# DiltheyLab/HLA-LA

Hardware: AMD Instinct MI355X
Metric: paired reads/sec aligned to PRG graph (higher is better)
Workload: dtype int32

## Files before the change

### hla-la_amd/__init__.py

```python
from __future__ import annotations

import ctypes as C
import os

import numpy as np

_HERE = os.path.dirname(os.path.abspath(__file__))
LIB_PATH = os.environ.get("HLALA_LIB_PATH") or os.path.join(_HERE, "libhlala_gpu.so")

c_i32p = C.POINTER(C.c_int32)
c_i64p = C.POINTER(C.c_int64)
c_u8p = C.POINTER(C.c_uint8)
c_u32p = C.POINTER(C.c_uint32)
c_f64p = C.POINTER(C.c_double)

CHAIN_OK, CHAIN_SKIP_STRAND, CHAIN_SKIP_DUP = 0, 1, 2
CHAIN_ERR_COLUMNS, CHAIN_ERR_FRONTIER, CHAIN_ERR_INPUT = -1, -2, -3


class GraphDesc(C.Structure):
    _fields_ = [("n_levels", C.c_int32), ("n_nodes", C.c_int32), ("n_edges", C.c_int32),
                ("node_level", c_i32p), ("edge_from", c_i32p), ("edge_to", c_i32p), ("edge_label", c_u8p)]


# ... 946 lines not shown
EXPORTED_SYMBOLS = [
    "hlala_debug_work_counters", "hlala_debug_dp_items", "hlala_debug_counters", "hlala_debug_buffer", "hlala_debug_memory",
    "hlala_set_tail_pool", "hlala_flush",
    "hlala_set_pair_overflow", "hlala_get_pair_overflow", "hlala_pair_overflow_need", "hlala_batch_get_pair_overflow",
    "hlala_comm_create", "hlala_comm_destroy", "hlala_comm_uses_rccl", "hlala_comm_last_error", "hlala_gather_pair_records", "hlala_reduce_coverage",
    "hlala_create", "hlala_destroy", "hlala_last_error", "hlala_graph_get_info", "hlala_graph_get_nodes",
    "hlala_graph_get_paths", "hlala_graph_get_gap_stretch", "hlala_batch_create",
    "hlala_batch_create_from_seeds", "hlala_batch_create_unpaired", "hlala_batch_set_first_chain", "hlala_batch_destroy", "hlala_project_chains", "hlala_extend_chains",
    "hlala_pair_chains", "hlala_align_batch", "hlala_batch_get_chains", "hlala_batch_get_pairs",
    "hlala_batch_get_stats", "hlala_batch_get_pairs_packed", "hlala_batch_export_pair_records", "hlala_set_gene_intervals", "hlala_postprocess_pairs", "hlala_get_coverage", "hlala_exon_loglik", "hlala_pair_loglik", "hlala_kat_phred",
    "hlala_kat_rand_r", "hlala_kat_exp", "hlala_abi_sizeof", "hlala_abi_version", "hlala_build_flags", "hlala_pack_bases", "hlala_call_locus", "hlala_exon_positions", "hlala_filter_positions", "hlala_estimate_insert_size", "hlala_graph_load_text", "hlala_graph_cache_save",
    "hlala_graph_cache_load", "hlala_graph_file_desc", "hlala_graph_file_free", "hlala_loader_last_error",
    "hlala_bam_extract_seeds", "hlala_bam_extract_seeds_mt", "hlala_bam_extract_seeds_opt", "hlala_seed_batch_counts", "hlala_seed_batch_desc", "hlala_seed_batch_window", "hlala_seed_batch_units", "hlala_seed_batch_name", "hlala_seed_batch_timing",
    "hlala_seed_batch_free", "hlala_seed_batch_pin", "hlala_bam_last_error", "hlala_bam_inflate_engine", "hlala_pinned_alloc", "hlala_pinned_free", "hlala_host_register", "hlala_host_unregister", "hlala_set_insert_size",
    "hlala_contigs_load_dir", "hlala_contigs_open_dir", "hlala_contigs_load_translations", "hlala_contigs_file_desc", "hlala_contigs_file_intervals", "hlala_contigs_file_free",
    "hlala_typer_open", "hlala_typer_close", "hlala_typer_last_error", "hlala_typer_n_levels", "hlala_typer_level_name", "hlala_typer_level_of", "hlala_typer_n_genes",
    "hlala_typer_gene", "hlala_typer_load_g_groups", "hlala_typer_g_translate", "hlala_typer_locus", "hlala_locus_free", "hlala_locus_get", "hlala_locus_cluster_id", "hlala_locus_type_cluster",
    "hlala_inflater_create", "hlala_inflater_destroy", "hlala_inflater_last_error", "hlala_bgzf_inflate", "hlala_bam_extract_seeds_gpu", "hlala_seed_batch_inflate_counts",
    "hlala_bgzf_inflate_crc", "hlala_seed_batch_crc_counts",
    "hlala_bam_scan", "hlala_bam_scan_status_text", "hlala_seed_batch_parse_counts", "hlala_seed_batch_transfer_bytes",
    "hlala_bam_group", "hlala_bam_group_rounds", "hlala_seed_batch_group_counts",
    "hlala_bam_name_order", "hlala_seed_batch_sort_counts",
    "hlala_bam_fill_create", "hlala_bam_fill_window", "hlala_bam_fill_last_error", "hlala_bam_fill_destroy", "hlala_seed_batch_fill_counts", "hlala_seed_batch_fill_ms",
    "hlala_batch_create_from_fill", "hlala_debug_batch_inputs",
    "hlala_locus_cluster_kmers", "hlala_type_locus", "hlala_kmer_presence", "hlala_kmer_keep_reads", "hlala_kmer_presence_kept", "hlala_kmer_forget_reads", "hlala_unit_alignment_stats", "hlala_typer_write_summary", "hlala_typer_begin_output", "hlala_locus_write_files", "hlala_locus_write_pairs_file", "hlala_typer_end_output",
]


PAIR_OVERFLOW_WAVES = 64


def pair_overflow_need(n1, n2, max_columns, unpaired=False):
    lib = load_library()
    lib.hlala_pair_overflow_need.argtypes = [C.c_int64, C.c_int64, C.c_int32, C.c_int]
    lib.hlala_pair_overflow_need.restype = C.c_int64
    return int(lib.hlala_pair_overflow_need(int(n1), int(n2), int(max_columns), int(bool(unpaired))))


class Context:

    def __init__(self, graph: dict, contigs: dict | None, insert_mean=200.0, insert_sd=35.0, rng_seed=12345,
                 long_read_mode=0, max_columns=384, device=0, stream=None):
        self.lib = load_library()
        self.max_columns = max_columns
        g, self._kg = fill_struct(GraphDesc, graph)
        self.params = Params(insert_mean, insert_sd, rng_seed, long_read_mode, max_columns, 0)
        h = C.c_void_p()
# ... 389 lines not shown
```

### hla-la_amd/csrc/hlala_api.hip

```cpp
#include <cmath>
#include <cstdio>
#include <cstring>
#include <cstdlib>
#include <algorithm>
#include <atomic>
#include <map>
#include <mutex>
#include <chrono>
#include <thread>
#include <set>
#include <string>
#include <unordered_map>
#include <vector>

#include "../../include/hlala_gpu.h"
#include "batch.h"
#include "flat_graph.hpp"
#include "host_internal.h"

#include "kernel_dp.hip"
#include "kernel_project.hip"
#include "kernel_order.hip"
#include "kernel_pair.hip"
#include "kernel_pair_overflow.hip"
// ... 14 lines not shown
size_t proj_slab_bytes_host(int stride, int maxNodesPerLevel) { return proj_slab_bytes(stride, maxNodesPerLevel); }
}

using namespace hlala;

static thread_local std::string g_create_error;

struct DevBuf {
    void* p = nullptr; size_t bytes = 0;
};

struct DpClass {
    int grid = 0, block = 0;
    char* slabs = nullptr; size_t slab_bytes = 0;
    const char* name = "";
    void (*launch)(hlala_ctx* c, const DpClass& k, hipStream_t ws, hlala_batch* b, const DpPoolArgs& pool) = nullptr;
};

struct hlala_ctx {
    int device = 0;
    hipStream_t stream = nullptr;
    hipStream_t side = nullptr;
    hipStream_t up = nullptr, rs = nullptr, active = nullptr;
    int tail_pool_k = 1; std::vector<hlala_batch*> tail;
    hipEvent_t evSideTail = nullptr; bool sideTailValid = false;
    hlala_params params{};
    FlatGraph F;
    DevGraph G{};
    DevGraph* dG = nullptr;
    DevTables* dT = nullptr;
    double* d_islog = nullptr;
    long long* d_contig_off = nullptr; uint8_t* d_contig_seq = nullptr; int* d_contig_level = nullptr;
    int n_contigs = 0; std::vector<long long> contig_off;
    std::vector<void*> allocs;
    std::unordered_map<void*, size_t> block_bytes;
    std::multimap<size_t, void*> pool;
    size_t pool_bytes = 0;
    size_t pool_cap = (size_t)176 << 30;
    std::mutex pool_mu;
    std::set<struct hlala_batch*> batches;
    int dp_long_bases = 48;
    int jf_margin = 16;
    int stitch_by_row = 1;
    int stitch_draw = 12;
    bool side_after_pair = false;
    bool rows_all = false;
// ... 145 lines not shown
    auto it = c->pool.lower_bound(bytes);
    if(it != c->pool.end() && it->first <= bytes + bytes / 4 + 4096) {
        *out = it->second; c->pool_bytes -= it->first; c->pool.erase(it);
        return 0;
    }
    void* p = nullptr;
    hipError_t e = device_malloc_retry(c->device, c, &p, bytes);
    if(e != hipSuccess) { c->err = std::string("hipMalloc: ") + hipGetErrorString(e); return HLALA_E_DEVICE; }
    c->block_bytes[p] = bytes;
    *out = p;
    return 0;
}
static void pool_release(hlala_ctx* c, void* p)
{
    if(!p) return;
    std::lock_guard<std::mutex> g(c->pool_mu);
    auto it = c->block_bytes.find(p);
    if(it == c->block_bytes.end()) { (void)hipFree(p); return; }
    if(c->pool_bytes + it->second > c->pool_cap) { c->block_bytes.erase(it); (void)hipFree(p); return; }
    c->pool.emplace(it->second, p); c->pool_bytes += it->second;
}

constexpr size_t PIN_GRANULE = (size_t)64 << 20;
template <class T>
static int dev_upload(hlala_ctx* c, std::vector<void*>& allocs, const T* host, size_t n, T** out)
{
    *out = nullptr;
    size_t bytes = (n ? n : 1) * sizeof(T);
    void* p = nullptr;
    { int rc_ = pool_malloc(c, &p, bytes); if(rc_) return rc_; }
    allocs.push_back(p);
    if(n && host) {
        const char* src = (const char*)host; char* dst = (char*)p; size_t left = n * sizeof(T);
        while(left) {
            const size_t toEdge = PIN_GRANULE - (size_t)((uintptr_t)src & (PIN_GRANULE - 1)), k = left < toEdge ? left : toEdge;
            HIP_TRY(c, hipMemcpyAsync(dst, src, k, hipMemcpyHostToDevice, c->active));
            src += k; dst += k; left -= k;
        }
    }
    *out = (T*)p;
    return 0;
}
template <class T>
static int dev_alloc(hlala_ctx* c, std::vector<void*>& allocs, size_t n, T** out, bool zero = false)
{
    *out = nullptr;
// ... 209 lines not shown
    c->proj_slab_bytes = proj_slab_bytes_host(c->params.max_columns, F.max_nodes_per_level);
    if(device_malloc_retry(c->device, nullptr, (void**)&c->proj_slabs, c->proj_slab_bytes * (size_t)c->proj_grid) != hipSuccess) { c->err = "hipMalloc(projection slabs) failed"; return fail(HLALA_E_DEVICE); }
    c->allocs.push_back(c->proj_slabs);
    if(!c->proj_long_slabs) {
        const char* e = getenv("HLALA_RETHREAD");
        if(!(e && atoi(e) == 0)) {
            size_t ent = (size_t)c->params.max_columns * (size_t)RT_SN; if(ent < 1024) ent = 1024;
            c->rethread_slab_bytes = (ent * sizeof(ChoiceRec) + 255) & ~(size_t)255;
            if(c->rethread_slab_bytes > c->proj_slab_bytes) c->rethread_slab_bytes = c->proj_slab_bytes;
            c->rethread_grid = cus * 24;
            if(device_malloc_retry(c->device, nullptr, (void**)&c->rethread_slabs, c->rethread_slab_bytes * (size_t)c->rethread_grid) != hipSuccess) { c->err = "hipMalloc(re-threading slabs) failed"; return fail(HLALA_E_DEVICE); }
            c->allocs.push_back(c->rethread_slabs);
        }
    }
    { const char* e = getenv("HLALA_LOCALITY");
      if(!(e && atoi(e) == 0)) { int sh = 8; if(e && atoi(e) >= 2 && atoi(e) <= 20) sh = atoi(e); while((F.L >> sh) + 2 > 16384) sh++; c->order_shift = sh; c->order_nb = (F.L >> sh) + 2; } }
    if(const char* e = getenv("HLALA_LONG_CHUNK_NODES")) { const int v = atoi(e); if(v >= 1) c->long_chunk_nodes = v; }
    if(const char* e = getenv("HLALA_LONG_MAXSEGS")) { const int v = atoi(e); if(v >= 0) c->long_max_segs = v; }
    if(c->proj_long_slabs && c->order_nb > 0) { const char* e = getenv("HLALA_LONG_ORDER"); c->order_cost = (e && atoi(e) == 0) ? 0 : 1; }
    if(getenv("HLALA_DEBUG")) { if(hipMalloc((void**)&c->dbg_host, 8192 * sizeof(int)) != hipSuccess) c->dbg_host = nullptr; else { (void)hipMemset(c->dbg_host, 0, 8192 * sizeof(int)); c->allocs.push_back(c->dbg_host); } }
    if(hipEventCreateWithFlags(&c->evSideTail, hipEventDisableTiming) != hipSuccess) { c->err = "hipEventCreate failed"; return fail(HLALA_E_DEVICE); }
    { int prLow = 0, prHigh = 0; (void)hipDeviceGetStreamPriorityRange(&prLow, &prHigh);
      if(hipStreamCreateWithPriority(&c->up, hipStreamNonBlocking, prHigh) != hipSuccess || hipStreamCreateWithPriority(&c->rs, hipStreamNonBlocking, prHigh) != hipSuccess ||
         hipStreamCreateWithPriority(&c->side, hipStreamNonBlocking, prLow) != hipSuccess) { c->err = "hipStreamCreate failed"; return fail(HLALA_E_DEVICE); } }
    if(hipStreamSynchronize(c->active) != hipSuccess) { c->err = "upload failed"; return fail(HLALA_E_DEVICE); }
    { std::lock_guard<std::mutex> g(g_ctx_mu); g_ctxs.push_back(c); }
    *out = c;
    return HLALA_OK;
}

void hlala_destroy(hlala_ctx* c)
{
    if(!c) return;
    DEV_GUARD(c);
    { std::lock_guard<std::mutex> g(g_ctx_mu); g_ctxs.erase(std::remove(g_ctxs.begin(), g_ctxs.end(), c), g_ctxs.end()); }
    if(!c->tail.empty()) (void)flush_tail(c);
    for(hlala_batch* b : c->batches) b->ctx = nullptr;
    for(void* p : c->allocs) if(p) (void)hipFree(p);
    if(c->pair_over_slabs) (void)hipFree(c->pair_over_slabs);
    if(c->create_scratch) { if(c->create_scratch_pinned) (void)hipHostFree(c->create_scratch); else free(c->create_scratch); }
    for(hlala_ctx::KeptReads& kr : c->kept) { (void)hipFree(kr.store); (void)hipFree(kr.start); (void)hipFree(kr.length); }
    for(auto& kv : c->pool) (void)hipFree(kv.second);
    if(c->side) { (void)hipStreamSynchronize(c->side); (void)hipStreamDestroy(c->side); }
    if(c->up) { (void)hipStreamSynchronize(c->up); (void)hipStreamDestroy(c->up); }
    if(c->rs) { (void)hipStreamSynchronize(c->rs); (void)hipStreamDestroy(c->rs); }
    if(c->evSideTail) (void)hipEventDestroy(c->evSideTail);
    delete c;
}

int hlala_graph_get_info(const hlala_ctx* c, hlala_graph_info* info)
{
    if(!c || !info) return HLALA_E_ARG;
    const FlatGraph& F = c->F;
    memset(info, 0, sizeof(*info));
    info->n_levels = F.L; info->n_nodes = F.N; info->n_edges = F.E; info->n_paths = (int)F.path_len.size();
    info->n_jump_entries = (int64_t)F.jf_node.size(); info->n_path_edges = (int64_t)F.path_edges.size();
    info->n_levelpos_entries = (int64_t)F.lp_seqid.size();
    info->max_nodes_per_level = F.max_nodes_per_level; info->max_out_degree = F.max_out_degree; info->max_in_degree = F.max_in_degree; info->max_jumps = F.max_jumps; info->max_parallel = F.max_parallel;
    for(uint8_t b : F.gap_stretch) info->n_gap_stretch_levels += b;
    return HLALA_OK;
}
int hlala_graph_get_nodes(const hlala_ctx* c, int32_t* node_orig, int32_t* level_off)
{
    if(!c) return HLALA_E_ARG;
    if(node_orig) memcpy(node_orig, c->F.node_orig.data(), c->F.node_orig.size() * 4);
    if(level_off) memcpy(level_off, c->F.level_off.data(), c->F.level_off.size() * 4);
    return HLALA_OK;
}
// ... 104 lines not shown
    DEV_GUARD(c);
    if(!c || !in || !out) return HLALA_E_ARG;
    UploadScope upscope_(c);
    *out = nullptr;
    if(in->n_pairs < 0 || in->n_chains < 0) { c->err = "negative batch sizes"; return HLALA_E_ARG; }
    if(!c->d_contig_off) { c->err = "hlala_batch_create needs contigs (hlala_create was called without them)"; return HLALA_E_STATE; }
    static const bool hostTiming = getenv("HLALA_HOST_TIMING") != nullptr;
    const auto tc0 = std::chrono::steady_clock::now(); auto tc1 = tc0, tc2 = tc0;
    hlala_batch* b = new hlala_batch(); b->ctx = c; c->batches.insert(b);
    DevBatch& B = b->B;
    B.n_pairs = in->n_pairs; B.n_reads = (unpaired ? 1 : 2) * in->n_pairs; B.n_chains = in->n_chains; B.stride = c->params.max_columns; B.from_seeds = 0; B.unpaired = unpaired ? 1 : 0;
    int nr = B.n_reads, nc = B.n_chains;
    auto fail = [&](int rc) { (void)hipStreamSynchronize(c->active); hlala_batch_destroy(b); return rc; };
    const int64_t rb0 = nr > 0 ? in->read_off[0] : 0, cb0 = nr > 0 ? in->chain_off[0] : 0;
    if(nr > 0) {
        const int64_t nbases64 = in->read_off[nr] - rb0, nc64 = in->chain_off[nr] - cb0;
        if(nbases64 < 0 || nc64 != (int64_t)nc || cb0 < 0 || rb0 < 0) { c->err = "inconsistent batch offsets"; return fail(HLALA_E_ARG); }
        if(nbases64 > 0x7FFFFFFFll) { c->err = "batch of " + std::to_string(nbases64) + " read bases: one batch holds at most 2^31 - 1 (cut the sample into more batches: hlala_seed_batch_window)"; return fail(HLALA_E_CAPACITY); }
    } else if(nc != 0) { c->err = "inconsistent batch offsets"; return fail(HLALA_E_ARG); }
    const int64_t gb0 = nc > 0 ? in->cigar_off[cb0] : 0;
    if(nc > 0) { const int64_t ng64 = in->cigar_off[cb0 + nc] - gb0; if(ng64 < 0) { c->err = "inconsistent batch offsets"; return fail(HLALA_E_ARG); }
                 if(ng64 > 0x7FFFFFFFll) { c->err = "batch of " + std::to_string(ng64) + " CIGAR operations: one batch holds at most 2^31 - 1"; return fail(HLALA_E_CAPACITY); } }
    b->first_chain = (uint32_t)cb0;
    int* chain_read = nullptr; int* read_off32 = nullptr; int* chain_off32 = nullptr; int* primary32 = nullptr; int* cigar_off32 = nullptr;
    {
        const size_t need = ((size_t)nc + (size_t)nr + 1 + (size_t)nr + 1 + (size_t)nr + (size_t)nc + 1 + 16) * sizeof(int);
        { const int rs = ctx_scratch(c, need); if(rs) return fail(rs); }
        int* q = (int*)c->create_scratch;
        chain_read = q; q += nc; read_off32 = q; q += (size_t)nr + 1; chain_off32 = q; q += (size_t)nr + 1; primary32 = q; q += nr; cigar_off32 = q;
    }
    const int32_t* w_contig = in->chain_contig + cb0; const int32_t* w_pos = in->chain_pos + cb0; const int32_t* w_offset = in->chain_offset + cb0; const int32_t* w_as = in->chain_as + cb0;
    const uint8_t* w_rev = in->chain_reverse + cb0;
    {
        struct Viol { long long at[5]; int kind1; };
        const int nt = (nr + nc) >= (1 << 18) ? 4 : 1;
        std::vector<Viol> viol((size_t)nt);
        const int n_contigs = c->n_contigs;
        auto work = [&](int t) {
            Viol v; for(int i = 0; i < 5; i++) v.at[i] = -1; v.kind1 = 0;
            const int r0 = (int)((long long)nr * t / nt), r1 = (int)((long long)nr * (t + 1) / nt);
            for(int r = r0; r < r1; r++) {
                const int64_t ro0 = in->read_off[r] - rb0, ro1 = in->read_off[r + 1] - rb0, co0 = in->chain_off[r] - cb0, co1 = in->chain_off[r + 1] - cb0;
                if((ro1 < ro0 || co1 < co0) && v.at[0] < 0) v.at[0] = r;
                read_off32[r] = (int)ro0; chain_off32[r] = (int)co0;
                int kind = 0;
                if((int)co1 <= (int)co0) kind = 1;
                else if((int)ro1 < (int)ro0) kind = 2;
                const int64_t pr = (int64_t)in->read_primary[r] - cb0;
                if(!kind && (pr < (int)co0 || pr >= (int)co1)) kind = 3;
                if(kind && v.at[1] < 0) { v.at[1] = r; v.kind1 = kind; }
                primary32[r] = (int)pr;
                if(co0 >= 0 && co1 <= (int64_t)nc) for(int64_t k = co0; k < co1; k++) chain_read[k] = r;
                if(!unpaired && (int)ro1 - (int)ro0 > DP_SEQCAP && v.at[4] < 0) v.at[4] = r;
            }
            const int k0 = (int)((long long)nc * t / nt), k1 = (int)((long long)nc * (t + 1) / nt);
            for(int k = k0; k < k1; k++) {
                if(in->cigar_off[cb0 + k + 1] < in->cigar_off[cb0 + k] && v.at[2] < 0) v.at[2] = k;
                cigar_off32[k] = (int)(in->cigar_off[cb0 + k] - gb0);
                if((w_contig[k] < 0 || w_contig[k] >= n_contigs) && v.at[3] < 0) v.at[3] = k;
            }
            viol[(size_t)t] = v;
        };
        if(nt == 1) work(0);
        else {
            std::vector<std::thread> th; int started = 0;
            try { th.reserve((size_t)nt); for(int t = 1; t < nt; t++) { th.emplace_back(work, t); started++; } } catch(...) { }
            work(0);
            for(int t = started + 1; t < nt; t++) work(t);
            for(std::thread& x : th) x.join();
        }
        if(nr > 0) { read_off32[nr] = (int)(in->read_off[nr] - rb0); chain_off32[nr] = (int)(in->chain_off[nr] - cb0); } else { read_off32[0] = 0; chain_off32[0] = 0; }
        if(nc > 0) cigar_off32[nc] = (int)(in->cigar_off[cb0 + nc] - gb0); else cigar_off32[0] = 0;
        long long first[5] = {-1, -1, -1, -1, -1}; int kind1 = 0;
        for(int t = 0; t < nt; t++) for(int i = 0; i < 5; i++) if(viol[(size_t)t].at[i] >= 0 && (first[i] < 0 || viol[(size_t)t].at[i] < first[i])) { first[i] = viol[(size_t)t].at[i]; if(i == 1) kind1 = viol[(size_t)t].kind1; }
        if(first[0] >= 0) { c->err = "inconsistent batch offsets"; return fail(HLALA_E_ARG); }
        if(first[1] >= 0) { c->err = kind1 == 1 ? "read without alignments" : (kind1 == 2 ? "inconsistent batch offsets" : "read_primary outside the read's chains"); return fail(HLALA_E_ARG); }
        if(first[2] >= 0) { c->err = "inconsistent batch offsets"; return fail(HLALA_E_ARG); }
        if(first[3] >= 0) { c->err = "chain_contig out of range"; return fail(HLALA_E_ARG); }
        if(first[4] >= 0) {
            const int r = (int)first[4];
            c->err = "paired read of " + std::to_string(read_off32[r + 1] - read_off32[r]) + " bases: the paired path holds reads of at most " + std::to_string(DP_SEQCAP) + " (use hlala_batch_create_unpaired for long reads)";
            return fail(HLALA_E_CAPACITY);
        }
    }
    size_t nbases = nr ? (size_t)read_off32[nr] : 0, ncig = nc ? (size_t)cigar_off32[nc] : 0;
    int rc = 0;
    tc1 = std::chrono::steady_clock::now();
#define UPB(field, ptr, n) do { rc = dev_upload(c, b->allocs, (ptr), (n), (std::remove_const<std::remove_pointer<decltype(B.field)>::type>::type**)&B.field); if(rc) return fail(rc); } while(0)
    UPB(read_off, read_off32, (size_t)nr + 1); UPB(read_quals, in->read_quals + rb0, nbases);
    if(in->read_bases_packed && nr > 0) {
        const int64_t R0 = in->first_read;
        if(R0 < 0) { c->err = "first_read is negative"; return fail(HLALA_E_ARG); }
        const int64_t p0 = (rb0 + R0 + 1) >> 1, p1 = ((in->read_off[nr] + R0 + (int64_t)nr + 1) >> 1) + 1;
        uint8_t* dPacked = nullptr; uint8_t* dBases = nullptr;
        rc = dev_upload(c, b->allocs, in->read_bases_packed + p0, (size_t)(p1 - p0), &dPacked); if(rc) return fail(rc);
        rc = dev_alloc(c, b->allocs, nbases, &dBases, false); if(rc) return fail(rc);
        hipLaunchKernelGGL(k_unpack_bases, dim3((unsigned)nr), dim3(64), 0, c->active, (const uint8_t*)dPacked, B.read_off, nr, (long long)rb0, (long long)R0, (long long)p0, dBases);
        { hipError_t el = hipGetLastError(); if(el != hipSuccess) { c->err = std::string("k_unpack_bases: ") + hipGetErrorString(el); return fail(HLALA_E_DEVICE); } }
        B.read_bases = dBases;
    } else {
        if(!in->read_bases && nbases > 0) { c->err = "neither read_bases nor read_bases_packed"; return fail(HLALA_E_ARG); }
        UPB(read_bases, in->read_bases + rb0, nbases);
    }
    UPB(chain_off, chain_off32, (size_t)nr + 1); UPB(read_primary, primary32, (size_t)nr);
    UPB(chain_read, chain_read, (size_t)nc);
    UPB(chain_contig, w_contig, (size_t)nc); UPB(chain_pos, w_pos, (size_t)nc); UPB(chain_offset, w_offset, (size_t)nc);
    UPB(chain_as, w_as, (size_t)nc); UPB(chain_reverse, w_rev, (size_t)nc);
    UPB(cigar_off, cigar_off32, (size_t)nc + 1); UPB(cigar, in->cigar + gb0, ncig);
#undef UPB
    rc = batch_create_tail(c, b, &tc2); if(rc) return fail(rc);
    if(hostTiming) { const auto tc3 = std::chrono::steady_clock::now(); auto ms = [](std::chrono::steady_clock::duration d) { return std::chrono::duration<double, std::milli>(d).count(); };
                     fprintf(stderr, "hlala_batch_create: checks and rebasing %.1f ms, allocations + uploads + kernels queued %.1f ms, waiting for the upload stream %.1f ms\n", ms(tc1 - tc0), ms(tc2 - tc1), ms(tc3 - tc2)); }
    *out = b;
    return HLALA_OK;
}

static int ensure_outputs(hlala_ctx* c, hlala_batch* b)
{
    if(b->outputs_ready) return HLALA_OK;
    int rc = batch_alloc_outputs(c, b); if(rc) return rc;
    HIP_TRY(c, hipMemcpyAsync(b->dB, &b->B, sizeof(DevBatch), hipMemcpyHostToDevice, c->active));
    b->outputs_ready = true;
    return HLALA_OK;
}

int hlala_batch_create_from_seeds(hlala_ctx* c, const hlala_seeds_in* in, hlala_batch** out)
{
    DEV_GUARD(c);
    if(!c || !in || !out) return HLALA_E_ARG;
    UploadScope upscope_(c);
    *out = nullptr;
    hlala_batch* b = new hlala_batch(); b->ctx = c; c->batches.insert(b);
    DevBatch& B = b->B;
    B.n_pairs = 0; B.n_reads = in->n_reads; B.n_chains = in->n_chains; B.stride = c->params.max_columns; B.from_seeds = 1;
    int nr = B.n_reads, nc = B.n_chains; int stride = B.stride;
// ... 427 lines not shown
            if(o->col_level && e == hipSuccess) e = hipMemcpyAsync(o->col_level + o0, dL, cols * 4, hipMemcpyDeviceToHost, c->active);
            if(o->col_edge && e == hipSuccess) e = hipMemcpyAsync(o->col_edge + o0, dE, cols * 4, hipMemcpyDeviceToHost, c->active);
            if(o->col_gchar && e == hipSuccess) e = hipMemcpyAsync(o->col_gchar + o0, dG, cols, hipMemcpyDeviceToHost, c->active);
            if(o->col_schar && e == hipSuccess) e = hipMemcpyAsync(o->col_schar + o0, dS, cols, hipMemcpyDeviceToHost, c->active);
            if(o->col_fromseed && e == hipSuccess) e = hipMemcpyAsync(o->col_fromseed + o0, dF, cols, hipMemcpyDeviceToHost, c->active);
            if(e == hipSuccess) e = hipStreamSynchronize(c->active);
            if(e != hipSuccess) { c->err = std::string("hlala_batch_get_pairs: ") + hipGetErrorString(e); return done(HLALA_E_DEVICE); }
        }
        done(0);
    }
    return HLALA_OK;
}

int hlala_batch_get_pairs_packed(hlala_ctx* c, hlala_batch* b, hlala_pairs_packed_out* o)
{
    DEV_GUARD(c);
    ReaderScope rscope_(c, b); if(rscope_.rc) return rscope_.rc;
    if(!c || !b || !o || !o->col_off) return HLALA_E_ARG;
    if(!(b->staged & 4)) { c->err = "pairs not computed"; return HLALA_E_STATE; }
    DevBatch& B = b->B;
    const size_t nr = (size_t)B.n_reads;
    o->n_cols_total = 0;
    if(nr == 0) { o->col_off[0] = 0; return HLALA_OK; }
    std::vector<void*> tmp;
    auto done = [&](int r_) { for(void* p : tmp) pool_release(c, p); return r_; };
    int rc = 0; long long *dN = nullptr, *dOff = nullptr; char* dCub = nullptr;
    if((rc = dev_alloc(c, tmp, nr + 1, &dN)) || (rc = dev_alloc(c, tmp, nr + 1, &dOff))) return done(rc);
    hipStream_t st = c->active;
    hipLaunchKernelGGL(k_selected_ncols, dim3((unsigned)((nr + 1 + 255) / 256)), dim3(256), 0, st, b->dB, (int)nr, dN);
    if((rc = check_launch(c, "k_selected_ncols"))) return done(rc);
    size_t cubBytes = 0;
    HIP_TRY_F(c, hipcub::DeviceScan::ExclusiveSum(nullptr, cubBytes, dN, dOff, (int)(nr + 1), st), done);
    if((rc = dev_alloc(c, tmp, cubBytes ? cubBytes : 1, &dCub))) return done(rc);
    HIP_TRY_F(c, hipcub::DeviceScan::ExclusiveSum(dCub, cubBytes, dN, dOff, (int)(nr + 1), st), done);
    long long total = 0;
    HIP_TRY_F(c, hipMemcpyAsync(&total, dOff + nr, sizeof(total), hipMemcpyDeviceToHost, st), done);
    HIP_TRY_F(c, hipStreamSynchronize(st), done);
    o->n_cols_total = total;
    { std::vector<long long> ho(nr + 1); if((rc = dl(c, ho.data(), dOff, nr + 1))) return done(rc); HIP_TRY_F(c, hipStreamSynchronize(st), done); for(size_t i = 0; i <= nr; i++) o->col_off[i] = ho[i]; }
    if(total > o->cap_cols) { c->err = "hlala_batch_get_pairs_packed: cap_cols too small (n_cols_total holds the need)"; return done(HLALA_E_CAPACITY); }
    if(total == 0) return done(HLALA_OK);
    int *dL = nullptr, *dE = nullptr; uint8_t *dG = nullptr, *dS = nullptr, *dF = nullptr, *dQ = nullptr;
    const size_t T = (size_t)total;
    if((o->col_level && (rc = dev_alloc(c, tmp, T, &dL))) || (o->col_edge && (rc = dev_alloc(c, tmp, T, &dE))) || (o->col_gchar && (rc = dev_alloc(c, tmp, T, &dG))) ||
       (o->col_schar && (rc = dev_alloc(c, tmp, T, &dS))) || (o->col_fromseed && (rc = dev_alloc(c, tmp, T, &dF))) || (o->col_mapq && (rc = dev_alloc(c, tmp, T, &dQ)))) return done(rc);
    const unsigned grid = (unsigned)std::min<size_t>(nr, (size_t)c->stitch_grid * 4);
    hipLaunchKernelGGL(k_gather_packed, dim3(grid), dim3(64), 0, st, b->dB, (int)nr, (const long long*)dOff, dL, dE, dG, dS, dF, dQ);
    if((rc = check_launch(c, "k_gather_packed"))) return done(rc);
    if((rc = dl(c, o->col_level, dL, T)) || (rc = dl(c, o->col_edge, dE, T)) || (rc = dl(c, o->col_gchar, dG, T)) || (rc = dl(c, o->col_schar, dS, T)) ||
       (rc = dl(c, o->col_fromseed, dF, T)) || (rc = dl(c, o->col_mapq, dQ, T))) return done(rc);
    HIP_TRY_F(c, hipStreamSynchronize(st), done);
    return done(HLALA_OK);
}

int hlala_estimate_insert_size(hlala_ctx* c, const hlala_batch_in* in, hlala_insert_size_out* out)
{
    DEV_GUARD(c);
    if(!c || !in || !out) return HLALA_E_ARG;
    memset(out, 0, sizeof(*out));
    const int np = in->n_pairs, nr = 2 * np;
    if(np <= 0) { c->err = "hlala_estimate_insert_size: no pairs"; return HLALA_E_ARG; }
    std::vector<int64_t> chain_off(nr + 1), cigar_off(nr + 1, 0); std::vector<int32_t> read_primary(nr), contig(nr), pos(nr), offset(nr), as(nr); std::vector<uint8_t> rev(nr); std::vector<uint32_t> cigar;
    for(int r = 0; r < nr; r++) {
        const int64_t ch = in->read_primary[r];
        if(ch < in->chain_off[r] || ch >= in->chain_off[r + 1]) { c->err = "read_primary outside the read's chains"; return HLALA_E_ARG; }
        chain_off[r] = r; read_primary[r] = r; contig[r] = in->chain_contig[ch]; pos[r] = in->chain_pos[ch]; offset[r] = in->chain_offset[ch]; as[r] = in->chain_as[ch]; rev[r] = in->chain_reverse[ch];
        cigar.insert(cigar.end(), in->cigar + in->cigar_off[ch], in->cigar + in->cigar_off[ch + 1]); cigar_off[r + 1] = (int64_t)cigar.size();
    }
    chain_off[nr] = nr;
    hlala_batch_in pb = *in;
    pb.chain_off = chain_off.data(); pb.read_primary = read_primary.data(); pb.n_chains = nr; pb.chain_contig = contig.data(); pb.chain_pos = pos.data();
    pb.chain_offset = offset.data(); pb.chain_as = as.data(); pb.chain_reverse = rev.data(); pb.cigar_off = cigar_off.data(); pb.cigar = cigar.data();
    hlala_batch* b = nullptr;
    int rc = hlala_batch_create(c, &pb, &b); if(rc) return rc;
    auto done = [&](int r_) { hlala_batch_destroy(b); return r_; };
// ... 2162 lines not shown
```

### hla-la_amd/csrc/kernel_order.hip

```cpp
#include "batch.h"

namespace hlala {

constexpr int ORDER_SCAN_THREADS = 1024;

__global__ __launch_bounds__(ORDER_SCAN_THREADS) void k_order_scan(int* hist, int nb)
{
    __shared__ int part[ORDER_SCAN_THREADS];
    const int t = threadIdx.x;
    const int per = (nb + ORDER_SCAN_THREADS - 1) / ORDER_SCAN_THREADS;
    const int a = t * per, z = min(nb, a + per);
    int s = 0;
    for(int i = a; i < z; i++) s += hist[i];
    part[t] = s;
    __syncthreads();
    for(int o = 1; o < ORDER_SCAN_THREADS; o <<= 1) {
        const int v = t >= o ? part[t - o] : 0;
        __syncthreads();
        part[t] += v;
        __syncthreads();
    }
    int run = part[t] - s;
    for(int i = a; i < z; i++) { const int h = hist[i]; hist[i] = run; run += h; }
}
// ... 8 lines not shown
    const int pos = atomicAdd(&B.order_hist[bk], 1);
    B.chain_order[pos] = c;
    if(B.chain_row) B.chain_row[c] = pos;
}

__global__ void k_unpack_bases(const uint8_t* __restrict__ packed, const int* __restrict__ read_off, const int n_reads, const long long rb0, const long long firstRead,
                               const long long p0, uint8_t* __restrict__ out)
{
    const int r = blockIdx.x;
    if(r >= n_reads) return;
    const int o0 = read_off[r], len = read_off[r + 1] - o0;
    const long long at = ((rb0 + (long long)o0 + firstRead + (long long)r + 1) >> 1) - p0;
    auto dec = [](unsigned c) -> uint8_t {
        const u32 w = c < 4 ? 0x4D43413Du : (c < 8 ? 0x56535247u : (c < 12 ? 0x48595754u : 0x4E42444Bu));
        return (uint8_t)(w >> (8 * (c & 3)));
    };
    for(int j = 2 * (int)threadIdx.x; j < len; j += 2 * (int)blockDim.x) {
        const unsigned b = packed[at + (j >> 1)];
        out[o0 + j] = dec(b >> 4);
        if(j + 1 < len) out[o0 + j + 1] = dec(b & 15u);
    }
}

}
```

### hla-la_amd/csrc/kernel_pair.hip

```cpp
#include "batch.h"
#include "../../include/hlala_gpu.h"

namespace hlala {

constexpr int PAIR_CHAINS = 64;
constexpr int PAIR_COMB   = 1024;
#ifndef HLALA_PAIR_COMB_LDS
#define HLALA_PAIR_COMB_LDS 128
#endif
constexpr int PAIR_COMB_LDS = HLALA_PAIR_COMB_LDS;
#ifndef PAIR_LEAN_WAVES
#define PAIR_LEAN_WAVES 6
#endif
#ifndef PAIR_MULTI_WAVES
#define PAIR_MULTI_WAVES 4
#endif
constexpr int PAIR_COLS   = 512;

constexpr short PAIR_NOCOL = -32768;
constexpr short PAIR_NOLEVEL = -32767;
struct __align__(16) PairListLds {
    int list[2][PAIR_CHAINS];
    int nlist[2];
    unsigned char src[2][PAIR_CHAINS];
// ... 582 lines not shown
    const int stride = B.stride;
    const int ch = B.best_chain[r];
    int n = 0;
    if(ch >= 0 && ch < B.n_chains) n = B.ext_ncols[ch];
    if(n < 0) n = 0;
    if(threadIdx.x == 0) oN[row] = n;
    const size_t so = (n > 0 ? row_base(B, ch) : (size_t)0), dofs = (size_t)row * stride;
    for(int j = threadIdx.x; j < stride; j += blockDim.x) {
        const bool in = j < n;
        oLevel[dofs + j] = in ? B.ext_level[so + j] : 0; oEdge[dofs + j] = in ? B.ext_edge[so + j] : 0;
        oG[dofs + j] = in ? B.ext_g[so + j] : 0; oS[dofs + j] = in ? B.ext_s[so + j] : 0; oFs[dofs + j] = in ? B.ext_fromseed[so + j] : 0;
    }
}

__global__ void k_selected_ncols(const DevBatch* __restrict__ Bp, int nReads, long long* __restrict__ n)
{
    const DevBatch& B = *Bp;
    const int r = blockIdx.x * blockDim.x + threadIdx.x;
    if(r > nReads) return;
    long long v = 0;
    if(r < nReads) { const int ch = B.best_chain[r]; if(ch >= 0 && ch < B.n_chains) { const int c = B.ext_ncols[ch]; if(c > 0) v = c; } }
    n[r] = v;
}
__global__ void k_gather_packed(const DevBatch* __restrict__ Bp, int nReads, const long long* __restrict__ off, int* __restrict__ oLevel, int* __restrict__ oEdge,
                                uint8_t* __restrict__ oG, uint8_t* __restrict__ oS, uint8_t* __restrict__ oFs, uint8_t* __restrict__ oMq)
{
    const DevBatch& B = *Bp;
    for(int r = blockIdx.x; r < nReads; r += gridDim.x) {
        const long long d0 = off[r]; const int n = (int)(off[r + 1] - d0);
        if(n <= 0) continue;
        const size_t so = row_base(B, B.best_chain[r]), mo = (size_t)r * B.stride;
        for(int j = threadIdx.x; j < n; j += blockDim.x) {
            if(oLevel) oLevel[d0 + j] = B.ext_level[so + j];
            if(oEdge) oEdge[d0 + j] = B.ext_edge[so + j];
            if(oG) oG[d0 + j] = B.ext_g[so + j];
            if(oS) oS[d0 + j] = B.ext_s[so + j];
            if(oFs) oFs[d0 + j] = B.ext_fromseed[so + j];
            if(oMq) oMq[d0 + j] = B.sel_mapq[mo + j];
        }
    }
}

__global__ void k_export_pairs(const DevBatch* __restrict__ Bp, double* out)
{
    const DevBatch& B = *Bp;
    int p = blockIdx.x * blockDim.x + threadIdx.x;
    if(p >= B.n_pairs) return;
    double* o = out + 8 * (size_t)p;
    if(B.unpaired) { o[0] = B.pair_status[p]; o[1] = B.best_chain[p]; o[2] = -1; o[3] = B.n_comb[p]; o[4] = B.pair_ll[p]; o[5] = B.pair_mapq[p]; o[6] = B.mate_mapq[p]; o[7] = 0; return; }
    o[0] = B.pair_status[p]; o[1] = B.best_chain[2 * p]; o[2] = B.best_chain[2 * p + 1]; o[3] = B.n_comb[p];
    o[4] = B.pair_ll[p]; o[5] = B.pair_mapq[p]; o[6] = B.mate_mapq[2 * p]; o[7] = B.mate_mapq[2 * p + 1];
}
// ... 3 lines not shown
```

### include/hlala_gpu.h

```cpp
#ifndef HLALA_GPU_H_
#define HLALA_GPU_H_

#include <stddef.h>
#include <stdint.h>

#ifdef __cplusplus
extern "C" {
#endif

#define HLALA_OK              0
#define HLALA_E_ARG          -1
#define HLALA_E_DEVICE       -2
#define HLALA_E_GRAPH        -3
#define HLALA_E_CAPACITY     -4
#define HLALA_E_STATE        -5

#define HLALA_CHAIN_OK             0
#define HLALA_CHAIN_SKIP_STRAND    1
#define HLALA_CHAIN_SKIP_DUP       2
#define HLALA_CHAIN_ERR_COLUMNS   -1
#define HLALA_CHAIN_ERR_FRONTIER  -2
#define HLALA_CHAIN_ERR_INPUT     -3

typedef struct {
// ... 550 lines not shown
int  hlala_locus_write_files(const hlala_locus* l, const hlala_locus_report_in* in, const char* out_dir, hlala_locus_report_out* out);
int  hlala_locus_write_pairs_file(const hlala_locus* l, int32_t n_clusters, const int32_t* order, const double* p_normalized, const double* pair_ll,
                                  const double* mis_avg, const char* out_dir);
int  hlala_typer_end_output(const char* out_dir, const char* loci_comma_separated, int32_t very_conservative_read_likelihoods);

int  hlala_kat_phred(hlala_ctx* ctx, int n, const double* p_correct, uint8_t* phred_out,
                     const uint8_t* phred_in, double* p_out);
int  hlala_kat_rand_r(hlala_ctx* ctx, int n, uint32_t* seeds_inout, int32_t* values_out);
int  hlala_kat_exp(hlala_ctx* ctx, int n, const double* x, double* exp_x);

int  hlala_abi_sizeof(const char* struct_name);

#define HLALA_ABI_VERSION 7
int  hlala_abi_version(void);
#define HLALA_DEBUG_WC_N           88
#define HLALA_DEBUG_WC_BAND_FETCH  48
#define HLALA_DEBUG_WC_BAND_WHY    62
#define HLALA_DEBUG_WC_BAND_TIED   68
int  hlala_debug_work_counters(hlala_ctx* ctx, hlala_batch* batch, int* out, int capacity);
int  hlala_debug_dp_items(hlala_ctx* ctx, hlala_batch* batch, int* items_out, long long items_capacity_bytes, int* retry_out, long long retry_capacity_bytes);
int  hlala_debug_counters(hlala_ctx* ctx, hlala_batch* batch, unsigned long long* out32);
int  hlala_debug_buffer(hlala_ctx* ctx, int* out8192, int clear);
int  hlala_debug_memory(hlala_ctx* ctx, hlala_batch* batch, unsigned long long* out4);

#define HLALA_BUILD_AGENT_RELEASE 2
int  hlala_build_flags(void);

#ifdef __cplusplus
}
#endif
#endif
```

Baseline: 5.733 million.

## Chunk packed-pair readback with double-buffered gather/copy overlap and early uploads

Packed-pair readback now gathers columns in chunks into two device buffer sets and copies each chunk to the host on a separate high-priority stream, so gather kernels overlap device-to-host copies. Batch creation queues the input uploads that need no host pass before the host validation loop, so they overlap the CPU checks. The per-chain read index is now built by a new GPU kernel instead of a host loop. Column offsets are copied straight into the output instead of through a temporary vector. The costs are more events and streams, per-chunk launch overhead, and a full stream synchronize on every exit path.

```diff
diff --git a/hla-la_amd/__init__.py b/hla-la_amd/__init__.py
--- a/hla-la_amd/__init__.py
+++ b/hla-la_amd/__init__.py
@@ -992,7 +992,7 @@
     "hlala_bam_group", "hlala_bam_group_rounds", "hlala_seed_batch_group_counts",
     "hlala_bam_name_order", "hlala_seed_batch_sort_counts",
     "hlala_bam_fill_create", "hlala_bam_fill_window", "hlala_bam_fill_last_error", "hlala_bam_fill_destroy", "hlala_seed_batch_fill_counts", "hlala_seed_batch_fill_ms",
-    "hlala_batch_create_from_fill", "hlala_debug_batch_inputs",
+    "hlala_batch_create_from_fill", "hlala_debug_batch_inputs", "hlala_debug_set_readback_chunk",
     "hlala_locus_cluster_kmers", "hlala_type_locus", "hlala_kmer_presence", "hlala_kmer_keep_reads", "hlala_kmer_presence_kept", "hlala_kmer_forget_reads", "hlala_unit_alignment_stats", "hlala_typer_write_summary", "hlala_typer_begin_output", "hlala_locus_write_files", "hlala_locus_write_pairs_file", "hlala_typer_end_output",
 ]
 
diff --git a/hla-la_amd/csrc/hlala_api.hip b/hla-la_amd/csrc/hlala_api.hip
--- a/hla-la_amd/csrc/hlala_api.hip
+++ b/hla-la_amd/csrc/hlala_api.hip
@@ -60,6 +60,7 @@
     hipStream_t stream = nullptr;
     hipStream_t side = nullptr;
     hipStream_t up = nullptr, rs = nullptr, active = nullptr;
+    hipStream_t rs_copy = nullptr; hipEvent_t evRbGather[2] = {nullptr, nullptr}, evRbCopy[2] = {nullptr, nullptr}; long long readback_chunk = 0;
     int tail_pool_k = 1; std::vector<hlala_batch*> tail;
     hipEvent_t evSideTail = nullptr; bool sideTailValid = false;
     hlala_params params{};
@@ -251,6 +252,7 @@
 }
 
 constexpr size_t PIN_GRANULE = (size_t)64 << 20;
+constexpr long long READBACK_CHUNK_DEFAULT = 32ll << 20;
 template <class T>
 static int dev_upload(hlala_ctx* c, std::vector<void*>& allocs, const T* host, size_t n, T** out)
 {
@@ -506,7 +508,8 @@
     if(hipEventCreateWithFlags(&c->evSideTail, hipEventDisableTiming) != hipSuccess) { c->err = "hipEventCreate failed"; return fail(HLALA_E_DEVICE); }
     { int prLow = 0, prHigh = 0; (void)hipDeviceGetStreamPriorityRange(&prLow, &prHigh);
       if(hipStreamCreateWithPriority(&c->up, hipStreamNonBlocking, prHigh) != hipSuccess || hipStreamCreateWithPriority(&c->rs, hipStreamNonBlocking, prHigh) != hipSuccess ||
-         hipStreamCreateWithPriority(&c->side, hipStreamNonBlocking, prLow) != hipSuccess) { c->err = "hipStreamCreate failed"; return fail(HLALA_E_DEVICE); } }
+         hipStreamCreateWithPriority(&c->side, hipStreamNonBlocking, prLow) != hipSuccess || hipStreamCreateWithPriority(&c->rs_copy, hipStreamNonBlocking, prHigh) != hipSuccess) { c->err = "hipStreamCreate failed"; return fail(HLALA_E_DEVICE); } }
+    for(int s = 0; s < 2; s++) if(hipEventCreateWithFlags(&c->evRbGather[s], hipEventDisableTiming) != hipSuccess || hipEventCreateWithFlags(&c->evRbCopy[s], hipEventDisableTiming) != hipSuccess) { c->err = "hipEventCreate failed"; return fail(HLALA_E_DEVICE); }
     if(hipStreamSynchronize(c->active) != hipSuccess) { c->err = "upload failed"; return fail(HLALA_E_DEVICE); }
     { std::lock_guard<std::mutex> g(g_ctx_mu); g_ctxs.push_back(c); }
     *out = c;
@@ -528,6 +531,8 @@
     if(c->side) { (void)hipStreamSynchronize(c->side); (void)hipStreamDestroy(c->side); }
     if(c->up) { (void)hipStreamSynchronize(c->up); (void)hipStreamDestroy(c->up); }
     if(c->rs) { (void)hipStreamSynchronize(c->rs); (void)hipStreamDestroy(c->rs); }
+    if(c->rs_copy) { (void)hipStreamSynchronize(c->rs_copy); (void)hipStreamDestroy(c->rs_copy); }
+    for(int s = 0; s < 2; s++) { if(c->evRbGather[s]) (void)hipEventDestroy(c->evRbGather[s]); if(c->evRbCopy[s]) (void)hipEventDestroy(c->evRbCopy[s]); }
     if(c->evSideTail) (void)hipEventDestroy(c->evSideTail);
     delete c;
 }
@@ -678,15 +683,33 @@
     if(nc > 0) { const int64_t ng64 = in->cigar_off[cb0 + nc] - gb0; if(ng64 < 0) { c->err = "inconsistent batch offsets"; return fail(HLALA_E_ARG); }
                  if(ng64 > 0x7FFFFFFFll) { c->err = "batch of " + std::to_string(ng64) + " CIGAR operations: one batch holds at most 2^31 - 1"; return fail(HLALA_E_CAPACITY); } }
     b->first_chain = (uint32_t)cb0;
-    int* chain_read = nullptr; int* read_off32 = nullptr; int* chain_off32 = nullptr; int* primary32 = nullptr; int* cigar_off32 = nullptr;
+    int* read_off32 = nullptr; int* chain_off32 = nullptr; int* primary32 = nullptr; int* cigar_off32 = nullptr;
     {
-        const size_t need = ((size_t)nc + (size_t)nr + 1 + (size_t)nr + 1 + (size_t)nr + (size_t)nc + 1 + 16) * sizeof(int);
+        const size_t need = ((size_t)nr + 1 + (size_t)nr + 1 + (size_t)nr + (size_t)nc + 1 + 16) * sizeof(int);
         { const int rs = ctx_scratch(c, need); if(rs) return fail(rs); }
         int* q = (int*)c->create_scratch;
-        chain_read = q; q += nc; read_off32 = q; q += (size_t)nr + 1; chain_off32 = q; q += (size_t)nr + 1; primary32 = q; q += nr; cigar_off32 = q;
+        read_off32 = q; q += (size_t)nr + 1; chain_off32 = q; q += (size_t)nr + 1; primary32 = q; q += nr; cigar_off32 = q;
     }
     const int32_t* w_contig = in->chain_contig + cb0; const int32_t* w_pos = in->chain_pos + cb0; const int32_t* w_offset = in->chain_offset + cb0; const int32_t* w_as = in->chain_as + cb0;
     const uint8_t* w_rev = in->chain_reverse + cb0;
+    const size_t nbases = nr ? (size_t)(in->read_off[nr] - rb0) : 0, ncig = nc ? (size_t)(in->cigar_off[cb0 + nc] - gb0) : 0;
+    const bool packed = in->read_bases_packed && nr > 0;
+    const int argErr = packed ? (in->first_read < 0 ? 1 : 0) : (!in->read_bases && nbases > 0 ? 2 : 0);
+    int rc = 0; uint8_t* dPacked = nullptr; int64_t packed_p0 = 0; size_t bytesUp = 0;
+#define UPB(field, ptr, n) do { rc = dev_upload(c, b->allocs, (ptr), (n), (std::remove_const<std::remove_pointer<decltype(B.field)>::type>::type**)&B.field); if(rc) return fail(rc); bytesUp += (size_t)(n) * sizeof(*B.field); } while(0)
+    if(!argErr) {
+        UPB(read_quals, in->read_quals + rb0, nbases);
+        if(packed) {
+            const int64_t R0 = in->first_read;
+            const int64_t p0 = (rb0 + R0 + 1) >> 1, p1 = ((in->read_off[nr] + R0 + (int64_t)nr + 1) >> 1) + 1;
+            rc = dev_upload(c, b->allocs, in->read_bases_packed + p0, (size_t)(p1 - p0), &dPacked); if(rc) return fail(rc);
+            packed_p0 = p0; bytesUp += (size_t)(p1 - p0);
+        } else UPB(read_bases, in->read_bases + rb0, nbases);
+        UPB(chain_contig, w_contig, (size_t)nc); UPB(chain_pos, w_pos, (size_t)nc); UPB(chain_offset, w_offset, (size_t)nc);
+        UPB(chain_as, w_as, (size_t)nc); UPB(chain_reverse, w_rev, (size_t)nc);
+        UPB(cigar, in->cigar + gb0, ncig);
+    }
+    const auto tcq = std::chrono::steady_clock::now();
     {
         struct Viol { long long at[5]; int kind1; };
         const int nt = (nr + nc) >= (1 << 18) ? 4 : 1;
@@ -706,7 +729,6 @@
                 if(!kind && (pr < (int)co0 || pr >= (int)co1)) kind = 3;
                 if(kind && v.at[1] < 0) { v.at[1] = r; v.kind1 = kind; }
                 primary32[r] = (int)pr;
-                if(co0 >= 0 && co1 <= (int64_t)nc) for(int64_t k = co0; k < co1; k++) chain_read[k] = r;
                 if(!unpaired && (int)ro1 - (int)ro0 > DP_SEQCAP && v.at[4] < 0) v.at[4] = r;
             }
             const int k0 = (int)((long long)nc * t / nt), k1 = (int)((long long)nc * (t + 1) / nt);
@@ -739,34 +761,33 @@
             return fail(HLALA_E_CAPACITY);
         }
     }
-    size_t nbases = nr ? (size_t)read_off32[nr] : 0, ncig = nc ? (size_t)cigar_off32[nc] : 0;
-    int rc = 0;
+    if(argErr) { c->err = argErr == 1 ? "first_read is negative" : "neither read_bases nor read_bases_packed"; return fail(HLALA_E_ARG); }
     tc1 = std::chrono::steady_clock::now();
-#define UPB(field, ptr, n) do { rc = dev_upload(c, b->allocs, (ptr), (n), (std::remove_const<std::remove_pointer<decltype(B.field)>::type>::type**)&B.field); if(rc) return fail(rc); } while(0)
-    UPB(read_off, read_off32, (size_t)nr + 1); UPB(read_quals, in->read_quals + rb0, nbases);
-    if(in->read_bases_packed && nr > 0) {
-        const int64_t R0 = in->first_read;
-        if(R0 < 0) { c->err = "first_read is negative"; return fail(HLALA_E_ARG); }
-        const int64_t p0 = (rb0 + R0 + 1) >> 1, p1 = ((in->read_off[nr] + R0 + (int64_t)nr + 1) >> 1) + 1;
-        uint8_t* dPacked = nullptr; uint8_t* dBases = nullptr;
-        rc = dev_upload(c, b->allocs, in->read_bases_packed + p0, (size_t)(p1 - p0), &dPacked); if(rc) return fail(rc);
+    UPB(read_off, read_off32, (size_t)nr + 1);
+    if(packed) {
+        uint8_t* dBases = nullptr;
         rc = dev_alloc(c, b->allocs, nbases, &dBases, false); if(rc) return fail(rc);
-        hipLaunchKernelGGL(k_unpack_bases, dim3((unsigned)nr), dim3(64), 0, c->active, (const uint8_t*)dPacked, B.read_off, nr, (long long)rb0, (long long)R0, (long long)p0, dBases);
+        hipLaunchKernelGGL(k_unpack_bases, dim3((unsigned)nr), dim3(64), 0, c->active, (const uint8_t*)dPacked, B.read_off, nr, (long long)rb0, (long long)in->first_read, (long long)packed_p0, dBases);
         { hipError_t el = hipGetLastError(); if(el != hipSuccess) { c->err = std::string("k_unpack_bases: ") + hipGetErrorString(el); return fail(HLALA_E_DEVICE); } }
         B.read_bases = dBases;
-    } else {
-        if(!in->read_bases && nbases > 0) { c->err = "neither read_bases nor read_bases_packed"; return fail(HLALA_E_ARG); }
-        UPB(read_bases, in->read_bases + rb0, nbases);
     }
     UPB(chain_off, chain_off32, (size_t)nr + 1); UPB(read_primary, primary32, (size_t)nr);
-    UPB(chain_read, chain_read, (size_t)nc);
-    UPB(chain_contig, w_contig, (size_t)nc); UPB(chain_pos, w_pos, (size_t)nc); UPB(chain_offset, w_offset, (size_t)nc);
-    UPB(chain_as, w_as, (size_t)nc); UPB(chain_reverse, w_rev, (size_t)nc);
-    UPB(cigar_off, cigar_off32, (size_t)nc + 1); UPB(cigar, in->cigar + gb0, ncig);
+    UPB(cigar_off, cigar_off32, (size_t)nc + 1);
 #undef UPB
+    {
+        int* dChainRead = nullptr;
+        rc = dev_alloc(c, b->allocs, (size_t)nc, &dChainRead, false); if(rc) return fail(rc);
+        if(nr > 0 && nc > 0) {
+            hipLaunchKernelGGL(k_chain_read, dim3((unsigned)(((size_t)nr * 16 + 255) / 256)), dim3(256), 0, c->active, B.chain_off, nr, nc, dChainRead);
+            hipError_t el = hipGetLastError(); if(el != hipSuccess) { c->err = std::string("k_chain_read: ") + hipGetErrorString(el); return fail(HLALA_E_DEVICE); }
+        }
+        B.chain_read = dChainRead;
+    }
     rc = batch_create_tail(c, b, &tc2); if(rc) return fail(rc);
     if(hostTiming) { const auto tc3 = std::chrono::steady_clock::now(); auto ms = [](std::chrono::steady_clock::duration d) { return std::chrono::duration<double, std::milli>(d).count(); };
-                     fprintf(stderr, "hlala_batch_create: checks and rebasing %.1f ms, allocations + uploads + kernels queued %.1f ms, waiting for the upload stream %.1f ms\n", ms(tc1 - tc0), ms(tc2 - tc1), ms(tc3 - tc2)); }
+                     fprintf(stderr, "hlala_batch_create: uploads without a host pass queued %.1f ms, checks and rebasing %.1f ms, the rest of the allocations + uploads + kernels queued %.1f ms, "
+                                     "waiting for the upload stream %.1f ms, total %.1f ms, %zu bytes uploaded (%.1f GB/s over the total)\n",
+                             ms(tcq - tc0), ms(tc1 - tcq), ms(tc2 - tc1), ms(tc3 - tc2), ms(tc3 - tc0), bytesUp, (double)bytesUp / (ms(tc3 - tc0) * 1e6)); }
     *out = b;
     return HLALA_OK;
 }
@@ -1240,35 +1261,100 @@
     const size_t nr = (size_t)B.n_reads;
     o->n_cols_total = 0;
     if(nr == 0) { o->col_off[0] = 0; return HLALA_OK; }
-    std::vector<void*> tmp;
-    auto done = [&](int r_) { for(void* p : tmp) pool_release(c, p); return r_; };
+    static const bool hostTiming = getenv("HLALA_HOST_TIMING") != nullptr;
+    const auto t0 = std::chrono::steady_clock::now(); auto t1 = t0, t2 = t0, t3 = t0;
+    auto ms = [](std::chrono::steady_clock::duration d) { return std::chrono::duration<double, std::milli>(d).count(); };
+    hipStream_t st = c->active, cp = c->rs_copy;
+    std::vector<void*> tmp; size_t poolTaken = 0;
+    hipEvent_t evT[4] = {nullptr, nullptr, nullptr, nullptr};
+    auto done = [&](int r_) {
+        (void)hipStreamSynchronize(st); (void)hipStreamSynchronize(cp);
+        for(void* p : tmp) pool_release(c, p);
+        for(hipEvent_t e : evT) if(e) (void)hipEventDestroy(e);
+        return r_;
+    };
+    auto taken = [&](void* p) { std::lock_guard<std::mutex> g(c->pool_mu); auto it = c->block_bytes.find(p); if(it != c->block_bytes.end()) poolTaken += it->second; };
     int rc = 0; long long *dN = nullptr, *dOff = nullptr; char* dCub = nullptr;
     if((rc = dev_alloc(c, tmp, nr + 1, &dN)) || (rc = dev_alloc(c, tmp, nr + 1, &dOff))) return done(rc);
-    hipStream_t st = c->active;
     hipLaunchKernelGGL(k_selected_ncols, dim3((unsigned)((nr + 1 + 255) / 256)), dim3(256), 0, st, b->dB, (int)nr, dN);
     if((rc = check_launch(c, "k_selected_ncols"))) return done(rc);
     size_t cubBytes = 0;
     HIP_TRY_F(c, hipcub::DeviceScan::ExclusiveSum(nullptr, cubBytes, dN, dOff, (int)(nr + 1), st), done);
     if((rc = dev_alloc(c, tmp, cubBytes ? cubBytes : 1, &dCub))) return done(rc);
     HIP_TRY_F(c, hipcub::DeviceScan::ExclusiveSum(dCub, cubBytes, dN, dOff, (int)(nr + 1), st), done);
-    long long total = 0;
-    HIP_TRY_F(c, hipMemcpyAsync(&total, dOff + nr, sizeof(total), hipMemcpyDeviceToHost, st), done);
+    if(hostTiming) { HIP_TRY_F(c, hipStreamSynchronize(st), done); t1 = std::chrono::steady_clock::now(); }
+    static_assert(sizeof(long long) == sizeof(int64_t), "col_off is copied as it is scanned");
+    HIP_TRY_F(c, hipMemcpyAsync(o->col_off, dOff, (nr + 1) * sizeof(long long), hipMemcpyDeviceToHost, st), done);
     HIP_TRY_F(c, hipStreamSynchronize(st), done);
+    const int64_t* const off = o->col_off;
+    const long long total = off[nr];
     o->n_cols_total = total;
-    { std::vector<long long> ho(nr + 1); if((rc = dl(c, ho.data(), dOff, nr + 1))) return done(rc); HIP_TRY_F(c, hipStreamSynchronize(st), done); for(size_t i = 0; i <= nr; i++) o->col_off[i] = ho[i]; }
+    t2 = std::chrono::steady_clock::now();
     if(total > o->cap_cols) { c->err = "hlala_batch_get_pairs_packed: cap_cols too small (n_cols_total holds the need)"; return done(HLALA_E_CAPACITY); }
     if(total == 0) return done(HLALA_OK);
-    int *dL = nullptr, *dE = nullptr; uint8_t *dG = nullptr, *dS = nullptr, *dF = nullptr, *dQ = nullptr;
-    const size_t T = (size_t)total;
-    if((o->col_level && (rc = dev_alloc(c, tmp, T, &dL))) || (o->col_edge && (rc = dev_alloc(c, tmp, T, &dE))) || (o->col_gchar && (rc = dev_alloc(c, tmp, T, &dG))) ||
-       (o->col_schar && (rc = dev_alloc(c, tmp, T, &dS))) || (o->col_fromseed && (rc = dev_alloc(c, tmp, T, &dF))) || (o->col_mapq && (rc = dev_alloc(c, tmp, T, &dQ)))) return done(rc);
-    const unsigned grid = (unsigned)std::min<size_t>(nr, (size_t)c->stitch_grid * 4);
-    hipLaunchKernelGGL(k_gather_packed, dim3(grid), dim3(64), 0, st, b->dB, (int)nr, (const long long*)dOff, dL, dE, dG, dS, dF, dQ);
-    if((rc = check_launch(c, "k_gather_packed"))) return done(rc);
-    if((rc = dl(c, o->col_level, dL, T)) || (rc = dl(c, o->col_edge, dE, T)) || (rc = dl(c, o->col_gchar, dG, T)) || (rc = dl(c, o->col_schar, dS, T)) ||
-       (rc = dl(c, o->col_fromseed, dF, T)) || (rc = dl(c, o->col_mapq, dQ, T))) return done(rc);
-    HIP_TRY_F(c, hipStreamSynchronize(st), done);
+    long long CH = c->readback_chunk > 0 ? c->readback_chunk : READBACK_CHUNK_DEFAULT;
+    if(CH < (long long)B.stride) CH = B.stride;
+    const size_t nSet = (size_t)std::min<long long>(CH, total);
+    const size_t S4 = (nSet * 4 + 255) & ~(size_t)255, S1 = (nSet + 255) & ~(size_t)255;
+    const size_t setBytes = (o->col_level ? S4 : 0) + (o->col_edge ? S4 : 0) + (o->col_gchar ? S1 : 0) + (o->col_schar ? S1 : 0) + (o->col_fromseed ? S1 : 0) + (o->col_mapq ? S1 : 0);
+    if(!setBytes) return done(HLALA_OK);
+    struct Set { int *L = nullptr, *E = nullptr; uint8_t *G = nullptr, *S = nullptr, *F = nullptr, *Q = nullptr; } set[2];
+    const int nSets = total > CH ? 2 : 1;
+    for(int s = 0; s < nSets; s++) {
+        char* p = nullptr;
+        if((rc = dev_alloc(c, tmp, setBytes, &p))) return done(rc);
+        if(o->col_level) { set[s].L = (int*)p; p += S4; } if(o->col_edge) { set[s].E = (int*)p; p += S4; }
+        if(o->col_gchar) { set[s].G = (uint8_t*)p; p += S1; } if(o->col_schar) { set[s].S = (uint8_t*)p; p += S1; }
+        if(o->col_fromseed) { set[s].F = (uint8_t*)p; p += S1; } if(o->col_mapq) { set[s].Q = (uint8_t*)p; p += S1; }
+    }
+    if(hostTiming) { for(void* p : tmp) taken(p); for(hipEvent_t& e : evT) HIP_TRY_F(c, hipEventCreate(&e), done); }
+    size_t ra = 0; int k = 0;
+    while(ra < nr) {
+        const size_t rb = (size_t)(std::upper_bound(off + ra, off + nr + 1, off[ra] + CH) - off) - 1;
+        if(rb <= ra || rb > nr) { c->err = "hlala_batch_get_pairs_packed: a read with more than max_columns selected columns"; return done(HLALA_E_DEVICE); }
+        const long long base = off[ra]; const size_t cols = (size_t)(off[rb] - base);
+        if(cols > 0) {
+            const Set& W = set[k & 1];
+            if(k >= 2) HIP_TRY_F(c, hipStreamWaitEvent(st, c->evRbCopy[k & 1], 0), done);
+            if(k == 0 && hostTiming) HIP_TRY_F(c, hipEventRecord(evT[0], st), done);
+            const unsigned grid = (unsigned)std::min<size_t>(rb - ra, (size_t)c->stitch_grid * 4);
+            hipLaunchKernelGGL(k_gather_packed, dim3(grid), dim3(64), 0, st, b->dB, (int)ra, (int)rb, (const long long*)dOff, base, W.L, W.E, W.G, W.S, W.F, W.Q);
+            if((rc = check_launch(c, "k_gather_packed"))) return done(rc);
+            HIP_TRY_F(c, hipEventRecord(c->evRbGather[k & 1], st), done);
+            HIP_TRY_F(c, hipStreamWaitEvent(cp, c->evRbGather[k & 1], 0), done);
+            if(k == 0 && hostTiming) HIP_TRY_F(c, hipEventRecord(evT[2], cp), done);
+            c->active = cp;
+            if((rc = dl(c, o->col_level ? o->col_level + base : nullptr, (const int32_t*)W.L, cols)) || (rc = dl(c, o->col_edge ? o->col_edge + base : nullptr, (const int32_t*)W.E, cols)) ||
+               (rc = dl(c, o->col_gchar ? o->col_gchar + base : nullptr, (const uint8_t*)W.G, cols)) || (rc = dl(c, o->col_schar ? o->col_schar + base : nullptr, (const uint8_t*)W.S, cols)) ||
+               (rc = dl(c, o->col_fromseed ? o->col_fromseed + base : nullptr, (const uint8_t*)W.F, cols)) || (rc = dl(c, o->col_mapq ? o->col_mapq + base : nullptr, (const uint8_t*)W.Q, cols))) { c->active = st; return done(rc); }
+            c->active = st;
+            HIP_TRY_F(c, hipEventRecord(c->evRbCopy[k & 1], cp), done);
+            k++;
+        }
+        ra = rb;
+    }
+    if(hostTiming) { HIP_TRY_F(c, hipEventRecord(evT[1], st), done); HIP_TRY_F(c, hipEventRecord(evT[3], cp), done); }
+    t3 = std::chrono::steady_clock::now();
+    HIP_TRY_F(c, hipStreamSynchronize(st), done); HIP_TRY_F(c, hipStreamSynchronize(cp), done);
+    if(hostTiming) {
+        const auto t4 = std::chrono::steady_clock::now();
+        float gms = 0, cms = 0; (void)hipEventElapsedTime(&gms, evT[0], evT[1]); (void)hipEventElapsedTime(&cms, evT[2], evT[3]);
+        const size_t perCol = (o->col_level ? 4 : 0) + (o->col_edge ? 4 : 0) + (o->col_gchar ? 1 : 0) + (o->col_schar ? 1 : 0) + (o->col_fromseed ? 1 : 0) + (o->col_mapq ? 1 : 0);
+        const double bytes = (double)total * (double)perCol + (double)(nr + 1) * 8.0;
+        fprintf(stderr, "hlala_batch_get_pairs_packed: count + scan %.1f ms, offsets %.1f ms, %d chunks of %lld columns queued %.1f ms, gathers %.1f ms (first to last, reader stream), "
+                        "copies %.1f ms (first to last, copy stream), total %.1f ms, %.0f bytes moved (%.1f GB/s over the total), %zu pool bytes taken\n",
+                ms(t1 - t0), ms(t2 - t1), k, CH, ms(t3 - t2), (double)gms, (double)cms, ms(t4 - t0), bytes, bytes / (ms(t4 - t0) * 1e6), poolTaken);
+    }
     return done(HLALA_OK);
+}
+
+int hlala_debug_set_readback_chunk(hlala_ctx* c, int64_t columns)
+{
+    if(!c) return HLALA_E_ARG;
+    if(columns <= 0) { c->readback_chunk = 0; return HLALA_OK; }
+    if(columns < (long long)c->params.max_columns) { c->err = "hlala_debug_set_readback_chunk: a chunk holds at least max_columns columns (one read always fits)"; return HLALA_E_ARG; }
+    c->readback_chunk = columns;
+    return HLALA_OK;
 }
 
 int hlala_estimate_insert_size(hlala_ctx* c, const hlala_batch_in* in, hlala_insert_size_out* out)
diff --git a/hla-la_amd/csrc/kernel_order.hip b/hla-la_amd/csrc/kernel_order.hip
--- a/hla-la_amd/csrc/kernel_order.hip
+++ b/hla-la_amd/csrc/kernel_order.hip
@@ -54,4 +54,13 @@
     }
 }
 
+__global__ __launch_bounds__(256) void k_chain_read(const int* __restrict__ chain_off, const int n_reads, const int n_chains, int* __restrict__ chain_read)
+{
+    const long long t = (long long)blockIdx.x * 256 + threadIdx.x, r = t >> 4;
+    if(r >= n_reads) return;
+    const int c0 = chain_off[r], c1 = chain_off[r + 1];
+    if(c0 < 0 || c1 > n_chains) return;
+    for(int k = c0 + (int)(threadIdx.x & 15u); k < c1; k += 16) chain_read[k] = (int)r;
 }
+
+}
diff --git a/hla-la_amd/csrc/kernel_pair.hip b/hla-la_amd/csrc/kernel_pair.hip
--- a/hla-la_amd/csrc/kernel_pair.hip
+++ b/hla-la_amd/csrc/kernel_pair.hip
@@ -628,12 +628,12 @@
     if(r < nReads) { const int ch = B.best_chain[r]; if(ch >= 0 && ch < B.n_chains) { const int c = B.ext_ncols[ch]; if(c > 0) v = c; } }
     n[r] = v;
 }
-__global__ void k_gather_packed(const DevBatch* __restrict__ Bp, int nReads, const long long* __restrict__ off, int* __restrict__ oLevel, int* __restrict__ oEdge,
+__global__ void k_gather_packed(const DevBatch* __restrict__ Bp, int r0, int r1, const long long* __restrict__ off, long long base, int* __restrict__ oLevel, int* __restrict__ oEdge,
                                 uint8_t* __restrict__ oG, uint8_t* __restrict__ oS, uint8_t* __restrict__ oFs, uint8_t* __restrict__ oMq)
 {
     const DevBatch& B = *Bp;
-    for(int r = blockIdx.x; r < nReads; r += gridDim.x) {
-        const long long d0 = off[r]; const int n = (int)(off[r + 1] - d0);
+    for(int r = r0 + (int)blockIdx.x; r < r1; r += gridDim.x) {
+        const long long d0 = off[r] - base; const int n = (int)(off[r + 1] - off[r]);
         if(n <= 0) continue;
         const size_t so = row_base(B, B.best_chain[r]), mo = (size_t)r * B.stride;
         for(int j = threadIdx.x; j < n; j += blockDim.x) {
diff --git a/include/hlala_gpu.h b/include/hlala_gpu.h
--- a/include/hlala_gpu.h
+++ b/include/hlala_gpu.h
@@ -596,6 +596,7 @@
 int  hlala_debug_counters(hlala_ctx* ctx, hlala_batch* batch, unsigned long long* out32);
 int  hlala_debug_buffer(hlala_ctx* ctx, int* out8192, int clear);
 int  hlala_debug_memory(hlala_ctx* ctx, hlala_batch* batch, unsigned long long* out4);
+int  hlala_debug_set_readback_chunk(hlala_ctx* ctx, int64_t columns);
 
 #define HLALA_BUILD_AGENT_RELEASE 2
 int  hlala_build_flags(void);
```

Result: slower. 5.642 million (-1.6%).
